# wcq99681-svg/YOLO-AD-Refine

Hardware: AMD Instinct MI355X
Metric: images/sec whole-node (640x640) fwd+bwd, YOLO-AD-Refine-n at 1/2/4/8 GPU (higher is better)
Workload: dtype bf16; 1 GPU; yolo11-701-YOLO-AD-Refine.yaml (n) train step bs=64/GPU 640x640, synthetic COCO-shape labels, TAL+DFL+CIoU/NWD loss, SGD+EMA; global_batch=64, img=640, parallelism=dp1, nms=not in the train step (measured in the inference leg at validator settings)

## Files before the change

include/adr.h:

```cpp
#ifndef ADR_H_
#define ADR_H_
#include <stddef.h>
#include <stdint.h>

#ifdef __cplusplus
extern "C" {
#endif

#define ADR_ABI_VERSION 1

enum adr_status { ADR_OK = 0, ADR_ERR_BAD_ARG = 1, ADR_ERR_UNSUPPORTED = 2, ADR_ERR_LAUNCH = 3 };
enum adr_dtype { ADR_F32 = 0, ADR_BF16 = 1 };
enum adr_act { ADR_ACT_NONE = 0, ADR_ACT_SILU = 1, ADR_ACT_GELU = 2, ADR_ACT_RELU = 3, ADR_ACT_SIGMOID = 4,
               ADR_ACT_HSWISH = 5 };

int adr_abi_version(void);
const char* adr_last_error(void);
int adr_memset_zero(void* ptr, size_t bytes, void* stream);

typedef struct adr_conv_desc {
  int n, h, w, c;
  int x_cstride, x_coff;
  int k, r, s;
  int stride_h, stride_w, pad_h, pad_w;
// ... 169 lines not shown

int adr_pack_weight(int dtype, const float* src, void* dst, int K, int C, int Cp, int RS, int transpose_kc,
                    void* stream);
int adr_pack_weight2(int dtype, const float* src, void* krsc, void* crsk, int K, int Kp, int C, int Cp, int RS,
                     int transpose_kc, void* stream);
int adr_pack_chunk_size(void);
int adr_pack_weight2_batched(int dtype, const void* table, int nchunks, void* stream);
int adr_pack_tile_size(void);
int adr_pack_weight2_tiled(int dtype, const void* table, int ntiles, void* stream);
int adr_unpack_weight_grad(const float* src, float* dst, int K, int C, int Cp, int RS, int transpose_kc,
                           int accumulate, void* stream);
int adr_stem_fwd_tiles(int N, int Ho);
int adr_stem_conv_fwd(const float* img, int N, int H, int W, const float* w, int K, void* y, int ycs, float* stats,
                      void* stream);
size_t adr_stem_wgrad_workspace(int N, int H, int W, int K);
int adr_stem_conv_wgrad(const float* img, int N, int H, int W, const void* dy, int dcs, int K, float* dw,
                        int accumulate, float* ws, size_t ws_bytes, void* stream);
int adr_stem_conv_fwd_u8(const uint8_t* img, int N, int H, int W, const float* w, int K, void* y, int ycs,
                         float* stats, void* stream);
int adr_stem_conv_wgrad_u8(const uint8_t* img, int N, int H, int W, const void* dy, int dcs, int K, float* dw,
                           int accumulate, float* ws, size_t ws_bytes, void* stream);
int adr_image_to_nhwc(int dtype, const float* src, void* dst, int N, int C, int H, int W, int Cp, void* stream);
int adr_image_u8_to_nhwc(int dtype, const uint8_t* src, void* dst, int N, int C, int H, int W, int Cp, void* stream);
int adr_cast(int src_dtype, const void* src, int dst_dtype, void* dst, long n, void* stream);

int adr_ew(int dtype, int op, int act, const void* a, int acs, const void* b, int bcs, const void* c, int ccs,
           void* o, int ocs, long npix, int C, const float* ca, const float* cb, int accumulate, void* stream);
int adr_bcast_mul(int dtype, const void* x, int xcs, const float* g, int gns, int gcs, const void* res, int rcs,
                  void* o, int ocs, int N, int HW, int C, int accumulate, void* stream);
int adr_dot_reduce(int dtype, const void* x, int xcs, const void* dz, int dcs, int N, int HW, int C,
                   int rows_per_chunk, float* partial, void* stream);
int adr_nc_collapse(const float* partial, int N, int chunks, int C, int which, float* out, int sum_n, int sum_c,
                    int accumulate, void* stream);
int adr_axpy(long n, float a, const float* x, float* y, void* stream);
typedef struct {
  const float* x;
  float* y;
  long n;
} adr_axpy_entry;
int adr_axpy_batched(const adr_axpy_entry* entries, int count, void* stream);
typedef struct adr_copy_piece {
  const void* src;
  void* dst;
  int scs, dcs, C, pad_;
} adr_copy_piece;
int adr_copy_pieces(const adr_copy_piece* pieces, int count, long npix, void* stream);
int adr_fusion_weights(const float* fw, int n, float eps, float* w, void* stream);
int adr_fusion_weights_bwd(const float* fw, int n, float eps, const float* dw, float* dfw, void* stream);

int adr_maxpool(int dtype, const void* x, int xcs, void* y, int ycs, uint8_t* arg, int N, int H, int W, int C, int k,
                void* stream);
int adr_maxpool_bwd(int dtype, const void* dy, int dcs, const uint8_t* arg, void* dx, int ocs, int N, int H, int W,
                    int C, int k, int accumulate, void* stream);
int adr_axis_mean(int dtype, const void* x, int xcs, int N, int H, int W, int C, void* oh, long ohn, void* ow,
                  long own, void* stream);
int adr_axis_mean_bwd(int dtype, const void* dh, long dhn, const void* dw, long dwn, void* dx, int ocs, int N, int H,
                      int W, int C, int accumulate, void* stream);
int adr_gate(int dtype, const void* x, int xcs, const void* ah, long ahn, const void* aw, long awn, void* o, int ocs,
             int N, int H, int W, int C, void* stream);
int adr_gate_bwd(int dtype, const void* x, int xcs, const void* ah, long ahn, const void* aw, long awn,
                 const void* dout, int dcs, void* dx, int ocs, void* dah, long dahn, void* daw, long dawn, int N,
                 int H, int W, int C, int accumulate, int zero_other, void* stream);
int adr_adapool(int dtype, const void* x, int xcs, int N, int H, int W, int C, void* y, int ycs, int OH, int OW,
                void* stream);
int adr_adapool_bwd(int dtype, const void* dy, int dcs, int N, int H, int W, int C, void* dx, int ocs, int OH, int OW,
                    int accumulate, void* stream);
int adr_bilinear(int dtype, const void* x, int xcs, int N, int H, int W, int C, void* y, int ycs, int OH, int OW,
                 void* stream);
int adr_bilinear_bwd(int dtype, const void* dy, int dcs, int N, int H, int W, int C, void* dx, int ocs, int OH,
                     int OW, int accumulate, void* stream);
int adr_upsample_nearest(int dtype, const void* x, int xcs, int N, int H, int W, int C, void* y, int ycs, int s,
                         void* stream);
int adr_upsample_nearest_bwd(int dtype, const void* dy, int dcs, int N, int H, int W, int C, void* dx, int ocs, int s,
                             int accumulate, void* stream);

int adr_mlca_fwd(int dtype, const void* y, int ycs, const void* res, int rcs, void* out, int ocs, int N, int H, int W,
                 int C, const float* wl, const float* wg, int k, float local_weight, float* local, float* att,
                 float* sig_l, float* sig_g, void* stream);
size_t adr_mlca_bwd_workspace(int N, int C, int k);
int adr_mlca_bwd(int dtype, const void* y, int ycs, const void* dout, int dcs, void* dy, int ocs, int N, int H, int W,
                 int C, const float* wl, const float* wg, int k, float local_weight, const float* local,
                 const float* att, const float* sig_l, const float* sig_g, float* dwl, float* dwg, float* ws,
                 size_t ws_bytes, void* stream);

int adr_dcn_im2col(int dtype, const void* x, int xcs, const void* om, int omcs, void* cols, int N, int H, int W,
                   int C, void* stream);
int adr_dcn_col2im(int dtype, const void* x, int xcs, const void* om, int omcs, const void* dcols, float* dx32,
                   void* dom, int domcs, int N, int H, int W, int C, int deterministic, void* stream);
int adr_dcn_fwd_bf16(const void* x, int xcs, const void* om, int omcs, const void* w_krsc, void* y, int ycs, int N,
                     int H, int W, int C, int Cout, void* stream);
int adr_dcn_wgrad_bf16_splits(int N, int H, int W, int C, int Cout);
int adr_dcn_wgrad_bf16(const void* x, int xcs, const void* om, int omcs, const void* dy, int dycs, float* part,
                       int splits, int N, int H, int W, int C, int Cout, void* stream);
int adr_dcn_bwd_bf16(const void* x, int xcs, const void* om, int omcs, const void* dy, int dycs, const void* w_t,
                     void* dx, int dxcs, void* dom, int domcs, float* dxf, int* tile_flags, int N, int H, int W, int C,
                     int Cout, void* stream);
int adr_dcn_bwd_tiles(int N, int H, int W);
typedef struct adr_dcn_level {
  const void* x;
  const void* om;
  const void* dy;
  void* y;
  void* dx;
  void* dom;
  float* dxf;
  int* flags;
// ... 152 lines not shown
```

yolo-ad-refine_amd/adrefine/kernels.py:

```python
from __future__ import annotations

import ctypes
import weakref

import torch

from .native import ConvDesc, lib

F32, BF16 = 0, 1
ACT = {"none": 0, "silu": 1, "gelu": 2, "relu": 3, "sigmoid": 4, "hswish": 5}
_NC_MIN_BLOCKS = int(__import__("os").environ.get("ADR_NC_MIN_BLOCKS", 512))
_NC_ROWS = int(__import__("os").environ.get("ADR_NC_ROWS", 1024))


def _stats_rows(N, HW):
    rows = _NC_ROWS
    if _NC_MIN_BLOCKS and N * -(-HW // rows) < _NC_MIN_BLOCKS:
        chunks = -(-_NC_MIN_BLOCKS // N)
        rows = max(32, -(-(-(-HW // chunks)) // 32) * 32)
    return rows


relayout_count = [0]
_TRACE_RELAYOUT = bool(int(__import__("os").environ.get("ADR_TRACE_RELAYOUT", "0")))
# ... 2243 lines not shown
        dxs = []
        for i, x in enumerate(xs):
            d = _new_like(x)
            _ew(EW_AXPBY, (d, d.data_ptr(), d.shape[1]), vd, vd, ca=w[i:i + 1], cb=z)
            dxs.append(d)
        dfw = torch.empty_like(fwd)
        if ctx.needs_input_grad[0] and all(_defer_dot(ctx.pfw, x, vd[0]) for x in xs):
            dwn = torch.empty(len(xs), dtype=torch.float32, device=dy.device)
            for i, x in enumerate(xs):
                _dfr().add_dotsum(x, vd[0], dwn[i:i + 1])
            n = fwd.numel()
            _dfr().post_dots.append(lambda: lib.adr_fusion_weights_bwd(fptr(fwd), n, 1e-4, fptr(dwn), fptr(dfw),
                                                                       stream()))
        else:
            dwn = torch.cat([_reduce_dot(x, vd[0], True, True) for x in xs])
            lib.adr_fusion_weights_bwd(fptr(fwd), fwd.numel(), 1e-4, fptr(dwn), fptr(dfw), stream())
        return (sink(ctx.pfw, dfw), *dxs)


def fusion(fw, xs):
    return FusionFn.apply(fw, *xs)




class MaxPoolFn(torch.autograd.Function):
    @staticmethod
    def forward(ctx, x, k, box=None):
        vx = _v(x)
        N, C, H, W = x.shape
        y, yp, ycs = _out_view(box, N, C, H, W, x.dtype, x.device)
        arg = torch.empty(N * H * W * C, dtype=torch.uint8, device=x.device)
        lib.adr_maxpool(dcode(x.dtype), ctypes.c_void_p(vx[1]), vx[2], ctypes.c_void_p(yp), ycs, fptr(arg),
                        N, H, W, C, k, stream())
        ctx.save_for_backward(arg)
        ctx.meta = (k, x.shape, x.dtype)
        ctx.sink = _sink_of(x)
        return y if box is None else y[:, :]

    @staticmethod
    def backward(ctx, dy):
        (arg,) = ctx.saved_tensors
        k, shape, dtype = ctx.meta
        N, C, H, W = shape
        vd = _v(dy)
        dx, acc = _dx_dst(ctx, (N, C, H, W), dtype, dy.device)
        lib.adr_maxpool_bwd(dcode(dtype), ctypes.c_void_p(vd[1]), vd[2], fptr(arg), ctypes.c_void_p(dx.data_ptr()),
                            dx.stride(3), N, H, W, C, k, acc, stream())
        return (None if ctx.sink is not None else dx), None, None


def maxpool(x, k, out=None):
    return MaxPoolFn.apply(x, k, None if out is None else OutBox(out))


class MLCAFn(torch.autograd.Function):

    @staticmethod
    def forward(ctx, y, res, wl, wg, local_weight, box=None):
        vy = _v(y)
        N, C, H, W = y.shape
        dev = y.device
        f = lambda *s: torch.empty(s, dtype=torch.float32, device=dev)
        local, att, sig_l, sig_g = f(N, 25, C), f(N, 25, C), f(N, 25 * C), f(N, C)
        out, op, ocs = _out_view(box, N, C, H, W, y.dtype, dev)
        vr = _v(res) if res is not None else None
        wlf, wgf = wl.detach().float().contiguous().view(-1), wg.detach().float().contiguous().view(-1)
        k = wlf.numel()
        lib.adr_mlca_fwd(dcode(y.dtype), ctypes.c_void_p(vy[1]), vy[2], ctypes.c_void_p(vr[1]) if vr else None,
                         vr[2] if vr else 0, ctypes.c_void_p(op), ocs, N, H, W, C, fptr(wlf), fptr(wgf), k,
                         float(local_weight), fptr(local), fptr(att), fptr(sig_l), fptr(sig_g), stream())
        ctx.save_for_backward(vy[0], wlf, wgf, local, att, sig_l, sig_g)
        ctx.meta = (local_weight, res is not None, wl.shape, wg.shape)
        ctx.pwl, ctx.pwg = wl, wg
        ctx.sres = getattr(res, "_adr_sink", None) if res is not None else None
        return out if box is None else out[:, :]

    @staticmethod
    def backward(ctx, dout):
        y, wlf, wgf, local, att, sig_l, sig_g = ctx.saved_tensors
        lw, has_res, wls, wgs = ctx.meta
        N, C, H, W = y.shape
        vd, vy = _v(dout), _v(y)
        dy = _new_like(y)
        k = wlf.numel()
        wsb = lib.adr_mlca_bwd_workspace(N, C, k)
        ws = torch.empty(wsb // 4 + 1, dtype=torch.float32, device=y.device)
        tl, tg = _target(ctx.pwl), _target(ctx.pwg)
        defer = (_DEFER_MLCA and _dfr() is not None and _TIMING is None and tl is not None and tg is not None
                 and tl is not tg)
        dwl = dwg = None
        if not defer:
            dwl = torch.empty(k, dtype=torch.float32, device=y.device)
            dwg = torch.empty(k, dtype=torch.float32, device=y.device)
        lib.adr_mlca_bwd(dcode(y.dtype), ctypes.c_void_p(vy[1]), vy[2], ctypes.c_void_p(vd[1]), vd[2],
                         ctypes.c_void_p(dy.data_ptr()), C, N, H, W, C, fptr(wlf), fptr(wgf), k, float(lw),
                         fptr(local), fptr(att), fptr(sig_l), fptr(sig_g), fptr(dwl), fptr(dwg), fptr(ws), wsb,
                         stream())
        dres = _defer_pass(ctx.sres, dout) if has_res else None
        if defer:
            rows = ws[2 * N * 25 * C:2 * N * 25 * C + 2 * N * k]
            for which, t in ((0, tl), (1, tg)):
                _dfr().add_psum(rows, N, k, which, fptr(_grad_buf(t)), 1)
                t._adr_used = True
            return dy, dres, None, None, None, None
        return dy, dres, sink(ctx.pwl, dwl.view(wls)), sink(ctx.pwg, dwg.view(wgs)), None, None
# ... 1853 lines not shown
```

yolo-ad-refine_amd/adrefine/native.py:

```python
from __future__ import annotations

import ctypes
import os
import re
from pathlib import Path

_HERE = Path(__file__).resolve().parent
LIB_PATH = Path(os.environ.get("ADR_LIB", _HERE / "lib" / "libadr_hip.so"))
HEADER = Path(os.environ["ADR_HEADER"]) if "ADR_HEADER" in os.environ else _HERE.parents[1] / "include" / "adr.h"
if not HEADER.exists():
    HEADER = _HERE / "lib" / "adr.h"


class ConvDesc(ctypes.Structure):
    _fields_ = [(n, ctypes.c_int) for n in (
        "n", "h", "w", "c", "x_cstride", "x_coff", "k", "r", "s", "stride_h", "stride_w", "pad_h", "pad_w",
        "ho", "wo", "y_cstride", "y_coff", "dtype")]


_STRUCTS = {"adr_conv_desc": ConvDesc}


def _ctype(t: str):
    t = t.replace("const", "").strip()
# ... 39 lines not shown
            fn.restype = ret
            fn.argtypes = args

    def __getattr__(self, name):
        fn = getattr(self.lib, name)
        ret = self.protos[name][0]
        if ret is ctypes.c_int and name not in _NONSTATUS:
            def call(*a):
                if OP_TRACE is not None:
                    return _traced(name, fn, a)
                if CALL_HOOK is not None:
                    return CALL_HOOK(name, fn, a)
                rc = fn(*a)
                if rc != 0:
                    raise RuntimeError(f"{name}: {self.lib.adr_last_error().decode()}")
                return rc
            setattr(self, name, call)
            return call
        setattr(self, name, fn)
        return fn


CALL_HOOK = None

OP_TRACE = None


def _traced(name, fn, a):
    import sys

    import torch
    e0, e1 = torch.cuda.Event(enable_timing=True), torch.cuda.Event(enable_timing=True)
    e0.record()
    rc = fn(*a)
    e1.record()
    if rc != 0:
        raise RuntimeError(f"{name}: {lib.lib.adr_last_error().decode()}")
    caller = f"{sys._getframe(2).f_code.co_name}<{sys._getframe(3).f_code.co_name}"
    ints = []
    for v in a:
        if isinstance(v, int) and not isinstance(v, bool) and abs(v) < (1 << 31):
            ints.append(v)
        elif isinstance(getattr(v, "_obj", None), ConvDesc):
            d = v._obj
            ints += [d.n, d.h, d.w, d.c, d.x_cstride, d.k, d.r, d.s, d.stride_h]
    ints = tuple(ints)
    OP_TRACE.append((name, caller, ints, e0, e1))
    return rc


_NONSTATUS = {"adr_abi_version", "adr_conv2d_wgrad_bias_fusable", "adr_dwconv_wgrad_bias_fusable", "adr_conv2d_fwd_stat_tiles", "adr_conv2d_fwd_bf16_stat_tiles", "adr_conv2d_wgrad_splits", "adr_nc_reduce_chunks", "adr_opt_entry_size", "adr_pack_chunk_size", "adr_pack_tile_size", "adr_stem_fwd_tiles",
              "adr_opt_chunk_size", "adr_dcn_wgrad_bf16_splits", "adr_gn_fused_supported",
              "adr_fp8_amax_blocks", "adr_conv2d_fp8_supported", "adr_conv2d_fwd_fp8_stat_tiles",
              "adr_dwconv_fwd_act_supported", "adr_dwconv_bwd_fused_supported", "adr_conv2d_bf16_xf_reuse", "adr_augment_desc_size",
              "adr_letterbox_desc_size", "adr_resize_desc_size", "adr_augment_mix_desc_size",
              "adr_dcn_bwd_tiles", "adr_conv2d_fwd_bf16_bnact_stat_tiles",
              "adr_conv2d_dgrad_bf16_stat_tiles", "adr_conv2d_wgrad_batched_tile", "adr_tta_view_size"}
_ = _NONSTATUS

lib = _Lib()
assert lib.lib.adr_abi_version() == 1, "ABI version mismatch"
```

yolo-ad-refine_amd/adrefine/nn/modules/block.py:

```python
from __future__ import annotations

import math

import torch
import torch.nn as nn

from ... import kernels as K
from .conv import Conv, Conv2d
from .mona import Mona

__all__ = ("Bottleneck", "C2f", "C3", "C3k", "C3k2", "SPPF", "MLCA", "Bottleneck_MLCA", "C3k_MLCA", "C3k2_MLCA",
           "ELA_HSFPN", "Multiply", "Add", "Fusion", "DFL", "Attention", "PSABlock", "C2PSA", "C2PTSSA", "DynamicTanh", "AttentionTSSA",
           "TSSAlock_DYT_Mona_EDFFN", "C2TSSA_DYT_Mona_EDFFN")


class Bottleneck(nn.Module):

    def __init__(self, c1, c2, shortcut=True, g=1, k=(3, 3), e=0.5):
        super().__init__()
        c_ = int(c2 * e)
        self.cv1 = Conv(c1, c_, k[0], 1)
        self.cv2 = Conv(c_, c2, k[1], 1, g=g)
        self.add = shortcut and c1 == c2

# ... 32 lines not shown
    def __init__(self, c1, c2, n=1, shortcut=True, g=1, e=0.5):
        super().__init__()
        c_ = int(c2 * e)
        self.cv1 = Conv(c1, c_, 1, 1)
        self.cv2 = Conv(c1, c_, 1, 1)
        self.cv3 = Conv(2 * c_, c2, 1)
        self.m = nn.Sequential(*(Bottleneck(c_, c_, shortcut, g, k=((1, 1), (3, 3)), e=1.0) for _ in range(n)))

    accepts_out = True

    def forward(self, x, out=None):
        xa, xb = K.fanout(x)
        N, _, H, W = x.shape
        c_ = self.cv1.conv.out_channels
        buf = K.empty_act(N, 2 * c_, H, W, x.dtype, x.device)
        *head, last = list(self.m)
        y = self.cv1(xa)
        for mm in head:
            y = mm(y)
        y = last(y, out=buf[:, :c_]) if getattr(last, "accepts_out", False) else last(y)
        return self.cv3(K.cat([y, self.cv2(xb, out=buf[:, c_:])], out=buf), out=out)


class C3k(C3):

    def __init__(self, c1, c2, n=1, shortcut=True, g=1, e=0.5, k=3):
        super().__init__(c1, c2, n, shortcut, g, e)
        c_ = int(c2 * e)
        self.m = nn.Sequential(*(Bottleneck(c_, c_, shortcut, g, k=(k, k), e=1.0) for _ in range(n)))


class C3k2(C2f):

    def __init__(self, c1, c2, n=1, c3k=False, e=0.5, g=1, shortcut=True):
        super().__init__(c1, c2, n, shortcut, g, e)
        self.m = nn.ModuleList(
            C3k(self.c, self.c, 2, shortcut, g) if c3k else Bottleneck(self.c, self.c, shortcut, g) for _ in range(n))


class SPPF(nn.Module):

    def __init__(self, c1, c2, k=5):
        super().__init__()
        c_ = c1 // 2
        self.cv1 = Conv(c1, c_, 1, 1)
        self.cv2 = Conv(c_ * 4, c2, 1, 1)
        self.k = k

    def forward(self, x, lazy=False):
        N, _, H, W = x.shape
        c_ = self.cv1.conv.out_channels
        buf = K.empty_act(N, 4 * c_, H, W, x.dtype, x.device)
        y = [self.cv1(x, out=buf[:, :c_])]
        for i in range(3):
            y[-1], feed = K.fanout(y[-1])
            y.append(K.maxpool(feed, self.k, out=buf[:, (i + 1) * c_:(i + 2) * c_]))
        return self.cv2(K.cat(y, out=buf), lazy=lazy)


class MLCA(nn.Module):

    def __init__(self, in_size, local_size=5, gamma=2, b=1, local_weight=0.5):
        super().__init__()
        if local_size != 5:
            raise NotImplementedError("libadr MLCA kernels are built for local_size=5 (the reference default)")
        self.local_size, self.gamma, self.b = local_size, gamma, b
        t = int(abs(math.log(in_size, 2) + self.b) / self.gamma)
        k = t if t % 2 else t + 1
        self.conv = nn.Conv1d(1, 1, kernel_size=k, padding=(k - 1) // 2, bias=False)
        self.conv_local = nn.Conv1d(1, 1, kernel_size=k, padding=(k - 1) // 2, bias=False)
        self.local_weight = local_weight

    def forward(self, x, res=None, out=None):
        return K.mlca(x, res, self.conv_local.weight, self.conv.weight, self.local_weight, out=out)


class Bottleneck_MLCA(Bottleneck):

    accepts_out = True

    def __init__(self, c1, c2, shortcut=True, g=1, k=(3, 3), e=0.5):
        super().__init__(c1, c2, shortcut, g, k, e)
        self.attention = MLCA(c2)

    def forward(self, x, out=None):
        if not self.add:
            return self.attention(self.cv2(self.cv1(x, lazy=True)), None, out=out)
        xa, xb = K.fanout(x)
        return self.attention(self.cv2(self.cv1(xa, lazy=True)), xb, out=out)


class C3k_MLCA(C3k):

    def __init__(self, c1, c2, n=1, shortcut=False, g=1, e=0.5, k=3):
        super().__init__(c1, c2, n, shortcut, g, e, k)
        c_ = int(c2 * e)
        self.m = nn.Sequential(*(Bottleneck_MLCA(c_, c_, shortcut, g, k=(k, k), e=1.0) for _ in range(n)))


class C3k2_MLCA(C3k2):

    def __init__(self, c1, c2, n=1, c3k=False, e=0.5, g=1, shortcut=True):
        super().__init__(c1, c2, n, c3k, e, g, shortcut)
        self.m = nn.ModuleList(C3k_MLCA(self.c, self.c, 2, shortcut, g) if c3k else
                               Bottleneck_MLCA(self.c, self.c, shortcut, g) for _ in range(n))

# ... 343 lines not shown
```

yolo-ad-refine_amd/csrc/adr_pool.hip:

```cpp
#include "adr_common.h"
#include <initializer_list>

namespace adr {

__device__ __forceinline__ int ad_start(int o, int in, int out) { return (int)(((long)o * in) / out); }
__device__ __forceinline__ int ad_end(int o, int in, int out) { return (int)(((long)(o + 1) * in + out - 1) / out); }

template <typename T, int VW>
__global__ void __launch_bounds__(256) maxpool_kernel(const T* x, int xcs, T* y, int ycs, uint8_t* arg, int N, int H,
                                                      int W, int C, int k) {
  const int G = C / VW;
  const PoolLanes L(G);
  if (!L.active) return;
  const long npix = (long)N * H * W;
  const int p = k / 2;
  POOL_LOOP(L, npix, G) {
    int n, h, w;
    pix_nhw(pix, H, W, n, h, w);
    const int c0 = cg * VW;
    float best[VW];
    int bi[VW];
#pragma unroll
    for (int e = 0; e < VW; ++e) {
      best[e] = -INFINITY;
// ... 2 lines not shown
    for (int dy = 0; dy < k; ++dy) {
      const int ih = h - p + dy;
      if (ih < 0 || ih >= H) continue;
      for (int dx = 0; dx < k; ++dx) {
        const int iw = w - p + dx;
        if (iw < 0 || iw >= W) continue;
        float v[VW];
        vload<T, VW>(x + (((long)n * H + ih) * W + iw) * xcs + c0, v);
#pragma unroll
        for (int e = 0; e < VW; ++e)
          if (v[e] > best[e] || isnan(v[e])) {
            best[e] = v[e];
            bi[e] = dy * k + dx;
          }
      }
    }
    vstore<T, VW>(y + pix * ycs + c0, best);
#pragma unroll
    for (int e = 0; e < VW; ++e) arg[pix * C + c0 + e] = (uint8_t)bi[e];
  }
}

template <typename T, int VW>
__global__ void __launch_bounds__(256) maxpool_bwd_kernel(const T* dy, int dcs, const uint8_t* arg, T* dx, int ocs,
                                                          int N, int H, int W, int C, int k, int accumulate) {
  const int G = C / VW;
  const PoolLanes L(G);
  if (!L.active) return;
  const long npix = (long)N * H * W;
  const int p = k / 2;
  POOL_LOOP(L, npix, G) {
    int n, h, w;
    pix_nhw(pix, H, W, n, h, w);
    const int c0 = cg * VW;
    float s[VW];
#pragma unroll
    for (int e = 0; e < VW; ++e) s[e] = 0.f;
    for (int oh = h - p; oh <= h + p; ++oh) {
      if (oh < 0 || oh >= H) continue;
      const int dyy = h - (oh - p);
      for (int ow = w - p; ow <= w + p; ++ow) {
        if (ow < 0 || ow >= W) continue;
        const int want = dyy * k + (w - (ow - p));
        const long o = ((long)n * H + oh) * W + ow;
        float g[VW];
        vload<T, VW>(dy + o * dcs + c0, g);
#pragma unroll
        for (int e = 0; e < VW; ++e)
          if (arg[o * C + c0 + e] == want) s[e] += g[e];
      }
    }
    vstore_acc<T, VW>(dx + pix * ocs + c0, s, accumulate);
  }
}

template <typename T, int VW>
__global__ void __launch_bounds__(256) axis_mean_kernel(const T* x, int xcs, int N, int H, int W, int C, T* oh,
                                                        long ohn, T* ow, long own) {
  __shared__ float red[256 * VW];
  const int n = blockIdx.y, b = blockIdx.x;
  const bool row = b < H;
  const int idx = row ? b : b - H;
  const int L = row ? W : H;
  const int G = C / VW;
  for (int cb = 0; cb < G; cb += 256) {
    const int gn = min(256, G - cb), S = 256 / gn;
    const int cg = cb + threadIdx.x % gn, sp = threadIdx.x / gn;
    float s[VW];
#pragma unroll
    for (int e = 0; e < VW; ++e) s[e] = 0.f;
    if (sp < S)
      for (int j = sp; j < L; j += S) {
        const int hh = row ? idx : j, ww = row ? j : idx;
        float v[VW];
        vload<T, VW>(x + (((long)n * H + hh) * W + ww) * xcs + cg * VW, v);
#pragma unroll
        for (int e = 0; e < VW; ++e) s[e] += v[e];
      }
#pragma unroll
    for (int e = 0; e < VW; ++e) red[threadIdx.x * VW + e] = s[e];
    __syncthreads();
    if (threadIdx.x < gn) {
      float t[VW];
#pragma unroll
      for (int e = 0; e < VW; ++e) t[e] = 0.f;
      for (int q = 0; q < S; ++q)
#pragma unroll
        for (int e = 0; e < VW; ++e) t[e] += red[(q * gn + threadIdx.x) * VW + e];
#pragma unroll
      for (int e = 0; e < VW; ++e) t[e] /= (float)L;
      T* dst = row ? oh + n * ohn + (long)idx * C : ow + n * own + (long)idx * C;
      vstore<T, VW>(dst + cg * VW, t);
    }
    __syncthreads();
  }
}

template <typename T, int VW>
__global__ void __launch_bounds__(256) axis_mean_bwd_kernel(const T* dh, long dhn, const T* dw, long dwn, T* dx,
                                                            int ocs, int N, int H, int W, int C, int accumulate) {
  const int G = C / VW;
  const PoolLanes L(G);
  if (!L.active) return;
  const long npix = (long)N * H * W;
  const float iw = 1.f / (float)W, ih = 1.f / (float)H;
  POOL_LOOP(L, npix, G) {
// ... 306 lines not shown

using namespace adr;

static bool vec_ok(int C, int vw, std::initializer_list<long> strides, std::initializer_list<const void*> ptrs) {
  if (C % vw) return false;
  for (long s : strides)
    if (s % vw) return false;
  for (const void* p : ptrs)
    if ((uintptr_t)p % 16) return false;
  return true;
}
static dim3 pool_grid(long npix, int G) {
  const long rpb = G <= 256 ? 256 / G : 1;
  long b = (npix + rpb - 1) / rpb;
  if (b > 65536) b = 65536;
  return dim3((unsigned)(b < 1 ? 1 : b));
}

#define P(t, x) ((t*)(x))
#define VW_OF(dtype) ((dtype) == ADR_BF16 ? 8 : 4)
#define GOF(dtype, vec, C) ((C) / ((vec) ? VW_OF(dtype) : 1))

extern "C" int adr_maxpool(int dtype, const void* x, int xcs, void* y, int ycs, uint8_t* arg, int N, int H, int W,
                           int C, int k, void* stream) {
  hipStream_t st = (hipStream_t)stream;
  ADR_REQUIRE(k % 2 == 1 && k * k <= 255, "maxpool: k=%d", k);
  const bool v = vec_ok(C, VW_OF(dtype), {xcs, ycs}, {x, y});
  const dim3 g = pool_grid((long)N * H * W, GOF(dtype, v, C));
  if (dtype == ADR_BF16) {
    if (v) hipLaunchKernelGGL((maxpool_kernel<__bf16, 8>), g, dim3(256), 0, st, P(const __bf16, x), xcs, P(__bf16, y), ycs, arg, N, H, W, C, k);
    else hipLaunchKernelGGL((maxpool_kernel<__bf16, 1>), g, dim3(256), 0, st, P(const __bf16, x), xcs, P(__bf16, y), ycs, arg, N, H, W, C, k);
  } else {
    if (v) hipLaunchKernelGGL((maxpool_kernel<float, 4>), g, dim3(256), 0, st, P(const float, x), xcs, P(float, y), ycs, arg, N, H, W, C, k);
    else hipLaunchKernelGGL((maxpool_kernel<float, 1>), g, dim3(256), 0, st, P(const float, x), xcs, P(float, y), ycs, arg, N, H, W, C, k);
  }
  return check_launch("adr_maxpool");
}

extern "C" int adr_maxpool_bwd(int dtype, const void* dy, int dcs, const uint8_t* arg, void* dx, int ocs, int N, int H,
                               int W, int C, int k, int accumulate, void* stream) {
  hipStream_t st = (hipStream_t)stream;
  const bool v = vec_ok(C, VW_OF(dtype), {dcs, ocs}, {dy, dx});
  const dim3 g = pool_grid((long)N * H * W, GOF(dtype, v, C));
  if (dtype == ADR_BF16) {
    if (v) hipLaunchKernelGGL((maxpool_bwd_kernel<__bf16, 8>), g, dim3(256), 0, st, P(const __bf16, dy), dcs, arg, P(__bf16, dx), ocs, N, H, W, C, k, accumulate);
    else hipLaunchKernelGGL((maxpool_bwd_kernel<__bf16, 1>), g, dim3(256), 0, st, P(const __bf16, dy), dcs, arg, P(__bf16, dx), ocs, N, H, W, C, k, accumulate);
  } else {
    if (v) hipLaunchKernelGGL((maxpool_bwd_kernel<float, 4>), g, dim3(256), 0, st, P(const float, dy), dcs, arg, P(float, dx), ocs, N, H, W, C, k, accumulate);
    else hipLaunchKernelGGL((maxpool_bwd_kernel<float, 1>), g, dim3(256), 0, st, P(const float, dy), dcs, arg, P(float, dx), ocs, N, H, W, C, k, accumulate);
  }
  return check_launch("adr_maxpool_bwd");
}

extern "C" int adr_axis_mean(int dtype, const void* x, int xcs, int N, int H, int W, int C, void* oh, long ohn,
                             void* ow, long own, void* stream) {
  hipStream_t st = (hipStream_t)stream;
  const bool v = vec_ok(C, VW_OF(dtype), {xcs, ohn, own}, {x, oh, ow});
  const dim3 g = dim3(H + W, N);
  if (dtype == ADR_BF16) {
    if (v) hipLaunchKernelGGL((axis_mean_kernel<__bf16, 8>), g, dim3(256), 0, st, P(const __bf16, x), xcs, N, H, W, C, P(__bf16, oh), ohn, P(__bf16, ow), own);
    else hipLaunchKernelGGL((axis_mean_kernel<__bf16, 1>), g, dim3(256), 0, st, P(const __bf16, x), xcs, N, H, W, C, P(__bf16, oh), ohn, P(__bf16, ow), own);
  } else {
    if (v) hipLaunchKernelGGL((axis_mean_kernel<float, 4>), g, dim3(256), 0, st, P(const float, x), xcs, N, H, W, C, P(float, oh), ohn, P(float, ow), own);
    else hipLaunchKernelGGL((axis_mean_kernel<float, 1>), g, dim3(256), 0, st, P(const float, x), xcs, N, H, W, C, P(float, oh), ohn, P(float, ow), own);
  }
  return check_launch("adr_axis_mean");
}

extern "C" int adr_axis_mean_bwd(int dtype, const void* dh, long dhn, const void* dw, long dwn, void* dx, int ocs,
                                 int N, int H, int W, int C, int accumulate, void* stream) {
  hipStream_t st = (hipStream_t)stream;
  const bool v = vec_ok(C, VW_OF(dtype), {dhn, dwn, ocs}, {dh, dw, dx});
  const dim3 g = pool_grid((long)N * H * W, GOF(dtype, v, C));
  if (dtype == ADR_BF16) {
    if (v) hipLaunchKernelGGL((axis_mean_bwd_kernel<__bf16, 8>), g, dim3(256), 0, st, P(const __bf16, dh), dhn, P(const __bf16, dw), dwn, P(__bf16, dx), ocs, N, H, W, C, accumulate);
    else hipLaunchKernelGGL((axis_mean_bwd_kernel<__bf16, 1>), g, dim3(256), 0, st, P(const __bf16, dh), dhn, P(const __bf16, dw), dwn, P(__bf16, dx), ocs, N, H, W, C, accumulate);
  } else {
    if (v) hipLaunchKernelGGL((axis_mean_bwd_kernel<float, 4>), g, dim3(256), 0, st, P(const float, dh), dhn, P(const float, dw), dwn, P(float, dx), ocs, N, H, W, C, accumulate);
    else hipLaunchKernelGGL((axis_mean_bwd_kernel<float, 1>), g, dim3(256), 0, st, P(const float, dh), dhn, P(const float, dw), dwn, P(float, dx), ocs, N, H, W, C, accumulate);
  }
  return check_launch("adr_axis_mean_bwd");
}

extern "C" int adr_gate(int dtype, const void* x, int xcs, const void* ah, long ahn, const void* aw, long awn, void* o,
                        int ocs, int N, int H, int W, int C, void* stream) {
  hipStream_t st = (hipStream_t)stream;
  const bool v = vec_ok(C, VW_OF(dtype), {xcs, ahn, awn, ocs}, {x, ah, aw, o});
  const dim3 g = pool_grid((long)N * H * W, GOF(dtype, v, C));
  if (dtype == ADR_BF16) {
    if (v) hipLaunchKernelGGL((gate_kernel<__bf16, 8>), g, dim3(256), 0, st, P(const __bf16, x), xcs, P(const __bf16, ah), ahn, P(const __bf16, aw), awn, P(__bf16, o), ocs, N, H, W, C);
    else hipLaunchKernelGGL((gate_kernel<__bf16, 1>), g, dim3(256), 0, st, P(const __bf16, x), xcs, P(const __bf16, ah), ahn, P(const __bf16, aw), awn, P(__bf16, o), ocs, N, H, W, C);
  } else {
    if (v) hipLaunchKernelGGL((gate_kernel<float, 4>), g, dim3(256), 0, st, P(const float, x), xcs, P(const float, ah), ahn, P(const float, aw), awn, P(float, o), ocs, N, H, W, C);
    else hipLaunchKernelGGL((gate_kernel<float, 1>), g, dim3(256), 0, st, P(const float, x), xcs, P(const float, ah), ahn, P(const float, aw), awn, P(float, o), ocs, N, H, W, C);
  }
  return check_launch("adr_gate");
}

extern "C" int adr_gate_bwd(int dtype, const void* x, int xcs, const void* ah, long ahn, const void* aw, long awn,
                            const void* dout, int dcs, void* dx, int ocs, void* dah, long dahn, void* daw, long dawn,
                            int N, int H, int W, int C, int accumulate, int zero_other, void* stream) {
  hipStream_t st = (hipStream_t)stream;
  const bool v = vec_ok(C, VW_OF(dtype), {xcs, ahn, awn, dcs, ocs, dahn, dawn}, {x, ah, aw, dout, dx, dah, daw});
  const dim3 g = dim3(H + W, N);
  if (dtype == ADR_BF16) {
    if (v) hipLaunchKernelGGL((gate_bwd_reduce_kernel<__bf16, 8>), g, dim3(256), 0, st, P(const __bf16, x), xcs, P(const __bf16, ah), ahn, P(const __bf16, aw), awn, P(const __bf16, dout), dcs, P(__bf16, dah), dahn, P(__bf16, daw), dawn, N, H, W, C, zero_other);
// ... 112 lines not shown
```

Before: 3285 images/s.

## Fuse SPPF's three chained maxpools into one LDS-resident kernel, fwd and bwd

Adds a single-launch SPPF pooling kernel that loads an 8-channel slice of the whole feature map into padded LDS, then runs the three chained k×k maxpools back to back in shared memory, writing outputs and argmax maps. The backward pass is fused the same way, accumulating the gradients of all three stages in LDS. The aim is to remove two extra launches each way and the global round-trips of the intermediate pool outputs and gradients. It is limited to bf16 maps small enough for 64KB LDS, and parallelism is only N×C/8 blocks, so occupancy may be low.

Result: no change. 3289 images/s (median of 6 runs) (+0.1%).

```diff
diff --git a/include/adr.h b/include/adr.h
--- a/include/adr.h
+++ b/include/adr.h
@@ -245,6 +245,12 @@
                 void* stream);
 int adr_maxpool_bwd(int dtype, const void* dy, int dcs, const uint8_t* arg, void* dx, int ocs, int N, int H, int W,
                     int C, int k, int accumulate, void* stream);
+int adr_sppf_pool_supported(int dtype, int H, int W, int C, int k, int cs);
+int adr_sppf_pool(const void* x, int xcs, void* y1, void* y2, void* y3, int ycs, uint8_t* arg1, uint8_t* arg2,
+                  uint8_t* arg3, int N, int H, int W, int C, int k, void* stream);
+int adr_sppf_pool_bwd(const void* g0, const void* g1, const void* g2, const void* g3, int gcs, const uint8_t* arg1,
+                      const uint8_t* arg2, const uint8_t* arg3, void* dx, int ocs, int N, int H, int W, int C, int k,
+                      void* stream);
 int adr_axis_mean(int dtype, const void* x, int xcs, int N, int H, int W, int C, void* oh, long ohn, void* ow,
                   long own, void* stream);
 int adr_axis_mean_bwd(int dtype, const void* dh, long dhn, const void* dw, long dwn, void* dx, int ocs, int N, int H,
diff --git a/yolo-ad-refine_amd/adrefine/kernels.py b/yolo-ad-refine_amd/adrefine/kernels.py
--- a/yolo-ad-refine_amd/adrefine/kernels.py
+++ b/yolo-ad-refine_amd/adrefine/kernels.py
@@ -2319,6 +2319,94 @@
 
 def maxpool(x, k, out=None):
     return MaxPoolFn.apply(x, k, None if out is None else OutBox(out))
+
+
+SPPF_PATH = {"fused": 0, "chain": 0}
+
+
+def sppf_fused_ok(dtype, H, W, C, k, cs):
+    return bool(dtype == torch.bfloat16 and _SEED_CAT and _FANOUT_SINK
+                and lib.adr_sppf_pool_supported(BF16, H, W, C, k, cs))
+
+
+def sppf_pool_raw(x, ys, k):
+    N, C, H, W = x.shape
+    vx = _v(x)
+    vy = [_v(y) for y in ys]
+    if vx[0] is not x or any(v[0] is not y for v, y in zip(vy, ys)) or len({v[2] for v in vy}) != 1:
+        raise RuntimeError("sppf_pool: NHWC views with one output channel stride expected")
+    args = [torch.empty(N * H * W * C, dtype=torch.uint8, device=x.device) for _ in range(3)]
+    if sppf_fused_ok(x.dtype, H, W, C, k, vx[2]) and vy[0][2] % 8 == 0:
+        SPPF_PATH["fused"] += 1
+        lib.adr_sppf_pool(ctypes.c_void_p(vx[1]), vx[2], ctypes.c_void_p(vy[0][1]), ctypes.c_void_p(vy[1][1]),
+                          ctypes.c_void_p(vy[2][1]), vy[0][2], fptr(args[0]), fptr(args[1]), fptr(args[2]),
+                          N, H, W, C, k, stream())
+    else:
+        SPPF_PATH["chain"] += 1
+        src = vx
+        for v, a in zip(vy, args):
+            lib.adr_maxpool(dcode(x.dtype), ctypes.c_void_p(src[1]), src[2], ctypes.c_void_p(v[1]), v[2], fptr(a),
+                            N, H, W, C, k, stream())
+            src = v
+    return args
+
+
+def sppf_pool_bwd_raw(gs, args, k, inplace=True):
+    N, C, H, W = gs[0].shape
+    vg = [_v(g) for g in gs]
+    if any(v[0] is not g for v, g in zip(vg, gs)) or len({v[2] for v in vg}) != 1:
+        raise RuntimeError("sppf_pool_bwd: NHWC views with one channel stride expected")
+    dt = gs[0].dtype
+    if sppf_fused_ok(dt, H, W, C, k, vg[0][2]):
+        SPPF_PATH["fused"] += 1
+        dx = gs[0] if inplace else _new_like(gs[0])
+        lib.adr_sppf_pool_bwd(ctypes.c_void_p(vg[0][1]), ctypes.c_void_p(vg[1][1]), ctypes.c_void_p(vg[2][1]),
+                              ctypes.c_void_p(vg[3][1]), vg[0][2], fptr(args[0]), fptr(args[1]), fptr(args[2]),
+                              ctypes.c_void_p(dx.data_ptr()), dx.stride(3), N, H, W, C, k, stream())
+        return dx
+    SPPF_PATH["chain"] += 1
+    if not inplace:
+        cp = []
+        for v in vg[:3]:
+            c = _new_like(v[0])
+            _ew(EW_COPY, (c, c.data_ptr(), C), v)
+            cp.append((c, c.data_ptr(), C))
+        vg = cp + [vg[3]]
+    for i in (2, 1, 0):
+        lib.adr_maxpool_bwd(dcode(dt), ctypes.c_void_p(vg[i + 1][1]), vg[i + 1][2], fptr(args[i]),
+                            ctypes.c_void_p(vg[i][1]), vg[i][2], N, H, W, C, k, 1, stream())
+    return vg[0][0]
+
+
+class SppfPoolFn(torch.autograd.Function):
+
+    @staticmethod
+    def forward(ctx, y0, k, box):
+        buf = box.t
+        N, c, H, W = y0.shape
+        v0 = _v(y0)
+        if tuple(buf.shape) != (N, 4 * c, H, W) or buf.stride(1) != 1 or buf.stride(3) != 4 * c or buf.dtype != y0.dtype:
+            raise RuntimeError("sppf_pool: buf must be a whole NHWC activation of four times y0's channels")
+        if not (v0[1] == buf.data_ptr() and v0[2] == 4 * c):
+            _ew(EW_COPY, (buf, buf.data_ptr(), 4 * c), v0)
+        args = sppf_pool_raw(buf[:, :c], [buf[:, (i + 1) * c:(i + 2) * c] for i in range(3)], k)
+        ctx.save_for_backward(*args)
+        ctx.meta = (k, c)
+        return buf[:, :]
+
+    @staticmethod
+    def backward(ctx, dy):
+        args = ctx.saved_tensors
+        k, c = ctx.meta
+        inplace = not getattr(dy, "_adr_pinned", False)
+        dy, _, _ = _v(dy)
+        dx = sppf_pool_bwd_raw([dy[:, i * c:(i + 1) * c] for i in range(4)], args, k, inplace=inplace)
+        dx._adr_excl = True
+        return dx, None, None
+
+
+def sppf_pool(y0, buf, k):
+    return SppfPoolFn.apply(y0, k, OutBox(buf))
 
 
 class MLCAFn(torch.autograd.Function):
diff --git a/yolo-ad-refine_amd/adrefine/native.py b/yolo-ad-refine_amd/adrefine/native.py
--- a/yolo-ad-refine_amd/adrefine/native.py
+++ b/yolo-ad-refine_amd/adrefine/native.py
@@ -115,7 +115,7 @@
 _NONSTATUS = {"adr_abi_version", "adr_conv2d_wgrad_bias_fusable", "adr_dwconv_wgrad_bias_fusable", "adr_conv2d_fwd_stat_tiles", "adr_conv2d_fwd_bf16_stat_tiles", "adr_conv2d_wgrad_splits", "adr_nc_reduce_chunks", "adr_opt_entry_size", "adr_pack_chunk_size", "adr_pack_tile_size", "adr_stem_fwd_tiles",
               "adr_opt_chunk_size", "adr_dcn_wgrad_bf16_splits", "adr_gn_fused_supported",
               "adr_fp8_amax_blocks", "adr_conv2d_fp8_supported", "adr_conv2d_fwd_fp8_stat_tiles",
-              "adr_dwconv_fwd_act_supported", "adr_dwconv_bwd_fused_supported", "adr_conv2d_bf16_xf_reuse", "adr_augment_desc_size",
+              "adr_dwconv_fwd_act_supported", "adr_dwconv_bwd_fused_supported", "adr_sppf_pool_supported", "adr_conv2d_bf16_xf_reuse", "adr_augment_desc_size",
               "adr_letterbox_desc_size", "adr_resize_desc_size", "adr_augment_mix_desc_size",
               "adr_dcn_bwd_tiles", "adr_conv2d_fwd_bf16_bnact_stat_tiles",
               "adr_conv2d_dgrad_bf16_stat_tiles", "adr_conv2d_wgrad_batched_tile", "adr_tta_view_size"}
diff --git a/yolo-ad-refine_amd/adrefine/nn/modules/block.py b/yolo-ad-refine_amd/adrefine/nn/modules/block.py
--- a/yolo-ad-refine_amd/adrefine/nn/modules/block.py
+++ b/yolo-ad-refine_amd/adrefine/nn/modules/block.py
@@ -108,6 +108,8 @@
         c_ = self.cv1.conv.out_channels
         buf = K.empty_act(N, 4 * c_, H, W, x.dtype, x.device)
         y = [self.cv1(x, out=buf[:, :c_])]
+        if K.sppf_fused_ok(y[0].dtype, H, W, c_, self.k, 4 * c_):
+            return self.cv2(K.sppf_pool(y[0], buf, self.k), lazy=lazy)
         for i in range(3):
             y[-1], feed = K.fanout(y[-1])
             y.append(K.maxpool(feed, self.k, out=buf[:, (i + 1) * c_:(i + 2) * c_]))
diff --git a/yolo-ad-refine_amd/csrc/adr_pool.hip b/yolo-ad-refine_amd/csrc/adr_pool.hip
--- a/yolo-ad-refine_amd/csrc/adr_pool.hip
+++ b/yolo-ad-refine_amd/csrc/adr_pool.hip
@@ -78,6 +78,149 @@
     }
     vstore_acc<T, VW>(dx + pix * ocs + c0, s, accumulate);
   }
+}
+
+constexpr int SPPF_CB = 8;
+typedef __attribute__((ext_vector_type(2))) unsigned int u32x2;
+__device__ __forceinline__ int sppf_rs(int W, int p) { return (W + 2 * p) | 1; }
+
+template <int KS>
+__device__ __forceinline__ void sppf_pool_stage(const u32x4* src, u32x4* dst, __bf16* y, int ycs, uint8_t* arg, int n,
+                                                int H, int W, int C, int c0, int k, int rs) {
+  const int kk = KS ? KS : k, p = kk / 2;
+  constexpr int UR = KS ? KS : 1;
+  for (int idx = threadIdx.x; idx < H * W; idx += 256) {
+    const int h = idx / W, w = idx - h * W;
+    float best[SPPF_CB];
+    int bi[SPPF_CB];
+#pragma unroll
+    for (int e = 0; e < SPPF_CB; ++e) {
+      best[e] = -INFINITY;
+      bi[e] = 0;
+    }
+#pragma unroll UR
+    for (int dy = 0; dy < kk; ++dy) {
+      const u32x4* row = src + (h + dy) * rs + w;
+#pragma unroll UR
+      for (int dx = 0; dx < kk; ++dx) {
+        const u32x4 v = row[dx];
+        const __bf16* ve = reinterpret_cast<const __bf16*>(&v);
+#pragma unroll
+        for (int e = 0; e < SPPF_CB; ++e) {
+          const float f = to_f(ve[e]);
+          if (f > best[e] || isnan(f)) {
+            best[e] = f;
+            bi[e] = dy * kk + dx;
+          }
+        }
+      }
+    }
+    u32x4 o;
+    __bf16* oe = reinterpret_cast<__bf16*>(&o);
+#pragma unroll
+    for (int e = 0; e < SPPF_CB; ++e) oe[e] = from_f<__bf16>(best[e]);
+    const long pix = ((long)n * H + h) * W + w;
+    st16(y + pix * ycs + c0, o);
+    if (dst) dst[(h + p) * rs + w + p] = o;
+    u32x2 a;
+    a[0] = (unsigned)bi[0] | (unsigned)bi[1] << 8 | (unsigned)bi[2] << 16 | (unsigned)bi[3] << 24;
+    a[1] = (unsigned)bi[4] | (unsigned)bi[5] << 8 | (unsigned)bi[6] << 16 | (unsigned)bi[7] << 24;
+    *reinterpret_cast<u32x2*>(arg + pix * C + c0) = a;
+  }
+}
+
+template <int KS>
+__global__ void __launch_bounds__(256) sppf_pool_kernel(const __bf16* x, int xcs, __bf16* y1, __bf16* y2, __bf16* y3,
+                                                        int ycs, uint8_t* a1, uint8_t* a2, uint8_t* a3, int H, int W,
+                                                        int C, int k) {
+  extern __shared__ __attribute__((aligned(16))) unsigned char sppf_sm[];
+  const int kk = KS ? KS : k, p = kk / 2, rs = sppf_rs(W, p), plane = (H + 2 * p) * rs;
+  const int n = blockIdx.x, c0 = blockIdx.y * SPPF_CB;
+  u32x4* pa = reinterpret_cast<u32x4*>(sppf_sm);
+  u32x4* pb = pa + plane;
+  const u32x4 ninf = {0xFF80FF80u, 0xFF80FF80u, 0xFF80FF80u, 0xFF80FF80u};
+  for (int i = threadIdx.x; i < 2 * plane; i += 256) pa[i] = ninf;
+  __syncthreads();
+  for (int idx = threadIdx.x; idx < H * W; idx += 256) {
+    const int h = idx / W, w = idx - h * W;
+    pa[(h + p) * rs + w + p] = ld16(x + (((long)n * H + h) * W + w) * xcs + c0);
+  }
+  __syncthreads();
+  sppf_pool_stage<KS>(pa, pb, y1, ycs, a1, n, H, W, C, c0, k, rs);
+  __syncthreads();
+  sppf_pool_stage<KS>(pb, pa, y2, ycs, a2, n, H, W, C, c0, k, rs);
+  __syncthreads();
+  sppf_pool_stage<KS>(pa, nullptr, y3, ycs, a3, n, H, W, C, c0, k, rs);
+}
+
+template <int KS>
+__device__ __forceinline__ void sppf_bwd_stage(const u32x4* src, const u32x2* ar, const __bf16* add, int acs,
+                                               u32x4* dst, __bf16* out, int ocs, int n, int H, int W, int c0, int k,
+                                               int rs) {
+  const int kk = KS ? KS : k, p = kk / 2;
+  constexpr int UR = KS ? KS : 1;
+  for (int idx = threadIdx.x; idx < H * W; idx += 256) {
+    const int h = idx / W, w = idx - h * W;
+    const long pix = ((long)n * H + h) * W + w;
+    const u32x4 av = ld16(add + pix * acs + c0);
+    float s[SPPF_CB];
+#pragma unroll
+    for (int e = 0; e < SPPF_CB; ++e) s[e] = 0.f;
+#pragma unroll UR
+    for (int a = 0; a < kk; ++a) {
+      const u32x4* srow = src + (h + a) * rs + w;
+      const u32x2* arow = ar + (h + a) * rs + w;
+#pragma unroll UR
+      for (int b = 0; b < kk; ++b) {
+        const unsigned want = (unsigned)((kk - 1 - a) * kk + (kk - 1 - b));
+        const u32x4 g = srow[b];
+        const u32x2 m = arow[b];
+        const __bf16* ge = reinterpret_cast<const __bf16*>(&g);
+#pragma unroll
+        for (int e = 0; e < SPPF_CB; ++e)
+          if (((m[e >> 2] >> (8 * (e & 3))) & 0xFFu) == want) s[e] += to_f(ge[e]);
+      }
+    }
+    const __bf16* ae = reinterpret_cast<const __bf16*>(&av);
+    u32x4 o;
+    __bf16* oe = reinterpret_cast<__bf16*>(&o);
+#pragma unroll
+    for (int e = 0; e < SPPF_CB; ++e) oe[e] = from_f<__bf16>(s[e] + to_f(ae[e]));
+    if (dst) dst[(h + p) * rs + w + p] = o;
+    else st16(out + pix * ocs + c0, o);
+  }
+}
+
+template <int KS>
+__global__ void __launch_bounds__(256) sppf_pool_bwd_kernel(const __bf16* g0, const __bf16* g1, const __bf16* g2,
+                                                            const __bf16* g3, int gcs, const uint8_t* a1,
+                                                            const uint8_t* a2, const uint8_t* a3, __bf16* dx, int ocs,
+                                                            int H, int W, int C, int k) {
+  extern __shared__ __attribute__((aligned(16))) unsigned char sppf_sm[];
+  const int kk = KS ? KS : k, p = kk / 2, rs = sppf_rs(W, p), plane = (H + 2 * p) * rs;
+  const int n = blockIdx.x, c0 = blockIdx.y * SPPF_CB;
+  u32x4* pa = reinterpret_cast<u32x4*>(sppf_sm);
+  u32x4* pb = pa + plane;
+  u32x2* ar = reinterpret_cast<u32x2*>(pb + plane);
+  const u32x4 z4 = {0u, 0u, 0u, 0u};
+  const u32x2 f2 = {0xFFFFFFFFu, 0xFFFFFFFFu};
+  for (int i = threadIdx.x; i < 2 * plane; i += 256) pa[i] = z4;
+  for (int i = threadIdx.x; i < 3 * plane; i += 256) ar[i] = f2;
+  __syncthreads();
+  for (int idx = threadIdx.x; idx < H * W; idx += 256) {
+    const int h = idx / W, w = idx - h * W, q = (h + p) * rs + w + p;
+    const long pix = ((long)n * H + h) * W + w;
+    pa[q] = ld16(g3 + pix * gcs + c0);
+    ar[q] = *reinterpret_cast<const u32x2*>(a1 + pix * C + c0);
+    ar[plane + q] = *reinterpret_cast<const u32x2*>(a2 + pix * C + c0);
+    ar[2 * plane + q] = *reinterpret_cast<const u32x2*>(a3 + pix * C + c0);
+  }
+  __syncthreads();
+  sppf_bwd_stage<KS>(pa, ar + 2 * plane, g2, gcs, pb, nullptr, 0, n, H, W, c0, k, rs);
+  __syncthreads();
+  sppf_bwd_stage<KS>(pb, ar + plane, g1, gcs, pa, nullptr, 0, n, H, W, c0, k, rs);
+  __syncthreads();
+  sppf_bwd_stage<KS>(pa, ar, g0, gcs, nullptr, dx, ocs, n, H, W, c0, k, rs);
 }
 
 template <typename T, int VW>
@@ -490,6 +633,69 @@
   return check_launch("adr_maxpool_bwd");
 }
 
+static bool sppf_env_on() {
+  const char* e = getenv("ADR_SPPF_FUSED");
+  return e ? atoi(e) != 0 : true;
+}
+static size_t sppf_smem(int H, int W, int k, bool bwd) {
+  const int p = k / 2;
+  const size_t plane = (size_t)(H + 2 * p) * ((W + 2 * p) | 1);
+  return plane * (bwd ? 2 * 16 + 3 * 8 : 2 * 16);
+}
+constexpr size_t SPPF_LDS_MAX = 64 * 1024;
+
+extern "C" int adr_sppf_pool_supported(int dtype, int H, int W, int C, int k, int cs) {
+  return sppf_env_on() && dtype == ADR_BF16 && C > 0 && C % SPPF_CB == 0 && cs % 8 == 0 && C / SPPF_CB <= 65535 &&
+                 H > 0 && W > 0 && k % 2 == 1 && k * k <= 255 && sppf_smem(H, W, k, true) <= SPPF_LDS_MAX
+             ? 1
+             : 0;
+}
+
+static bool al16(std::initializer_list<const void*> ptrs) {
+  for (const void* p : ptrs)
+    if (!p || (uintptr_t)p % 16) return false;
+  return true;
+}
+
+extern "C" int adr_sppf_pool(const void* x, int xcs, void* y1, void* y2, void* y3, int ycs, uint8_t* arg1,
+                             uint8_t* arg2, uint8_t* arg3, int N, int H, int W, int C, int k, void* stream) {
+  ADR_REQUIRE(adr_sppf_pool_supported(ADR_BF16, H, W, C, k, xcs) && ycs % 8 == 0 && N > 0,
+              "sppf_pool: N=%d H=%d W=%d C=%d k=%d not on the one-launch kernel", N, H, W, C, k);
+  ADR_REQUIRE(al16({x, y1, y2, y3}) && arg1 && arg2 && arg3 && (uintptr_t)arg1 % 8 == 0 && (uintptr_t)arg2 % 8 == 0 &&
+                  (uintptr_t)arg3 % 8 == 0,
+              "sppf_pool: pointers must be 16-byte (argmax maps 8-byte) aligned");
+  hipStream_t st = (hipStream_t)stream;
+  const dim3 g(N, C / SPPF_CB);
+  const size_t sm = sppf_smem(H, W, k, false);
+  if (k == 5)
+    hipLaunchKernelGGL((sppf_pool_kernel<5>), g, dim3(256), sm, st, P(const __bf16, x), xcs, P(__bf16, y1), P(__bf16, y2),
+                       P(__bf16, y3), ycs, arg1, arg2, arg3, H, W, C, k);
+  else
+    hipLaunchKernelGGL((sppf_pool_kernel<0>), g, dim3(256), sm, st, P(const __bf16, x), xcs, P(__bf16, y1), P(__bf16, y2),
+                       P(__bf16, y3), ycs, arg1, arg2, arg3, H, W, C, k);
+  return check_launch("adr_sppf_pool");
+}
+
+extern "C" int adr_sppf_pool_bwd(const void* g0, const void* g1, const void* g2, const void* g3, int gcs,
+                                 const uint8_t* arg1, const uint8_t* arg2, const uint8_t* arg3, void* dx, int ocs, int N,
+                                 int H, int W, int C, int k, void* stream) {
+  ADR_REQUIRE(adr_sppf_pool_supported(ADR_BF16, H, W, C, k, gcs) && ocs % 8 == 0 && N > 0,
+              "sppf_pool_bwd: N=%d H=%d W=%d C=%d k=%d not on the one-launch kernel", N, H, W, C, k);
+  ADR_REQUIRE(al16({g0, g1, g2, g3, dx}) && arg1 && arg2 && arg3 && (uintptr_t)arg1 % 8 == 0 &&
+                  (uintptr_t)arg2 % 8 == 0 && (uintptr_t)arg3 % 8 == 0,
+              "sppf_pool_bwd: pointers must be 16-byte (argmax maps 8-byte) aligned");
+  hipStream_t st = (hipStream_t)stream;
+  const dim3 g(N, C / SPPF_CB);
+  const size_t sm = sppf_smem(H, W, k, true);
+  if (k == 5)
+    hipLaunchKernelGGL((sppf_pool_bwd_kernel<5>), g, dim3(256), sm, st, P(const __bf16, g0), P(const __bf16, g1),
+                       P(const __bf16, g2), P(const __bf16, g3), gcs, arg1, arg2, arg3, P(__bf16, dx), ocs, H, W, C, k);
+  else
+    hipLaunchKernelGGL((sppf_pool_bwd_kernel<0>), g, dim3(256), sm, st, P(const __bf16, g0), P(const __bf16, g1),
+                       P(const __bf16, g2), P(const __bf16, g3), gcs, arg1, arg2, arg3, P(__bf16, dx), ocs, H, W, C, k);
+  return check_launch("adr_sppf_pool_bwd");
+}
+
 extern "C" int adr_axis_mean(int dtype, const void* x, int xcs, int N, int H, int W, int C, void* oh, long ohn,
                              void* ow, long own, void* stream) {
   hipStream_t st = (hipStream_t)stream;
```
